# junhuihe2000/FLGP

Hardware: AMD Instinct MI355X
Metric: points/sec through k-NN->Laplacian->trunc-SVD->heat-cov, n=1e6 d=16 K=200 (higher is better)
Workload: dtype f64

## Files before the change

flgp_amd/csrc/sparse.hip:

```cpp
#include "common.h"

namespace flgp {

__global__ __launch_bounds__(256) void csc_hist_kernel(const int *__restrict__ ell_idx, long nnz, int s,
                                                       int chunk, int *__restrict__ hist) {
  extern __shared__ int lh[];
  for (int j = threadIdx.x; j < s; j += blockDim.x) lh[j] = 0;
  __syncthreads();
  const long e0 = (long)blockIdx.x * chunk;
  long e1 = e0 + chunk;
  if (e1 > nnz) e1 = nnz;
  for (long e = e0 + threadIdx.x; e < e1; e += blockDim.x) atomicAdd(&lh[ell_idx[e]], 1);
  __syncthreads();
  int *out = hist + (size_t)blockIdx.x * s;
  for (int j = threadIdx.x; j < s; j += blockDim.x) out[j] = lh[j];
}

__global__ void csc_colscan_kernel(int *__restrict__ hist, int nchunks, int s, int *__restrict__ tot) {
  const int j = blockIdx.x * blockDim.x + threadIdx.x;
  if (j >= s) return;
  int run = 0;
  constexpr int CB = 16;
  int c = 0;
  for (; c + CB <= nchunks; c += CB) {
    int h[CB];
#pragma unroll
    for (int u = 0; u < CB; ++u) h[u] = hist[(size_t)(c + u) * s + j];
#pragma unroll
    for (int u = 0; u < CB; ++u) { hist[(size_t)(c + u) * s + j] = run; run += h[u]; }
  }
  for (; c < nchunks; ++c) {
    const int h = hist[(size_t)c * s + j];
    hist[(size_t)c * s + j] = run;
    run += h;
  }
  tot[j] = run;
}

__global__ __launch_bounds__(1024) void csc_scan_kernel(const int *__restrict__ tot, int s, int *__restrict__ colptr) {
  __shared__ int part[1024];
  const int t = threadIdx.x;
  const int per = (s + 1023) / 1024;
  const int lo = t * per, hi = (lo + per < s) ? lo + per : s;
  int sum = 0;
  for (int j = lo; j < hi; ++j) sum += tot[j];
  part[t] = sum;
  __syncthreads();
  for (int off = 1; off < 1024; off <<= 1) {
    int v = (t >= off) ? part[t - off] : 0;
    __syncthreads();
    part[t] += v;
    __syncthreads();
  }
  int run = (t == 0) ? 0 : part[t - 1];
  for (int j = lo; j < hi; ++j) { colptr[j] = run; run += tot[j]; }
  if (t == 1023) colptr[s] = part[1023];
}

__global__ __launch_bounds__(64) void csc_scatter_kernel(const int *__restrict__ ell_idx, long nnz, int s,
                                                         int chunk, int nbits, const int *__restrict__ hist,
                                                         const int *__restrict__ colptr, int *__restrict__ pos) {
  extern __shared__ int cur[];
  const int lane = threadIdx.x;
  for (int j = lane; j < s; j += 64) cur[j] = 0;
  __syncthreads();
  const int *hoff = hist + (size_t)blockIdx.x * s;
  const long e0 = (long)blockIdx.x * chunk;
  long e1 = e0 + chunk;
  if (e1 > nnz) e1 = nnz;
  const unsigned long long lt = (lane == 0) ? 0ull : (~0ull >> (64 - lane));
  for (long eb = e0; eb < e1; eb += 64) {
    const long e = eb + lane;
    const bool act = e < e1;
    const int col = act ? ell_idx[e] : 0;
    unsigned long long m = __ballot(act);
    for (int b = 0; b < nbits; ++b) {
      const bool bit = (col >> b) & 1;
      const unsigned long long bal = __ballot(bit);
      m &= bit ? bal : ~bal;
    }
    if (act) {
      const int rank = __popcll(m & lt);
      const int base = cur[col];
      pos[(size_t)colptr[col] + hoff[col] + base + rank] = (int)e;
      if (rank == 0) cur[col] = base + __popcll(m);
    }
    __syncthreads();
  }
}

constexpr int COLSUM_CHUNK = 1024;

template <bool WIN>
__global__ __launch_bounds__(64) void colsum_chunk_kernel(const int *__restrict__ ell_idx, const double *__restrict__ val,
                                                          int n, int r, int s, int nbits, double *__restrict__ part, int wmax,
                                                          int direct) {
  extern __shared__ double bins[];
  const int lane = threadIdx.x;
  const int w0 = WIN ? (int)blockIdx.y * wmax : 0;
  const int wn = WIN ? ((s - w0 < wmax) ? s - w0 : wmax) : s;
  for (int j = lane; j < wn; j += 64) bins[j] = 0.0;
  __syncthreads();
  const long i0 = (long)blockIdx.x * COLSUM_CHUNK;
  const long i1 = (i0 + COLSUM_CHUNK < n) ? i0 + COLSUM_CHUNK : n;
  const long e0 = i0 * r, e1 = i1 * r;
  if (direct) {
    constexpr int CU = 8;
    for (long eb = e0; eb < e1; eb += 64 * CU) {
      int cq[CU];
      double vq[CU];
#pragma unroll
      for (int u = 0; u < CU; ++u) {
        const long e = eb + 64 * u + lane;
        const long ec = e < e1 ? e : e1 - 1;
        cq[u] = ell_idx[ec];
        vq[u] = val[ec];
      }
#pragma unroll
      for (int u = 0; u < CU; ++u) {
        const bool on = eb + 64 * u + lane < e1 && (!WIN || (unsigned)(cq[u] - w0) < (unsigned)wn);
        const int bin = on ? cq[u] - w0 : 0;
        if (on) __builtin_amdgcn_ds_atomic_fadd_f64((__attribute__((address_space(3))) double *)&bins[bin], vq[u]);
      }
    }
    __syncthreads();
    double *outd = part + (size_t)blockIdx.x * s + w0;
    for (int j = lane; j < wn; j += 64) outd[j] = bins[j];
    return;
  }
  const unsigned long long lt = (lane == 0) ? 0ull : (~0ull >> (64 - lane));
  long e = e0 + lane;
  int col = (e < e1) ? ell_idx[e] : 0;
  double v = (e < e1) ? val[e] : 0.0;
  for (long eb = e0; eb < e1; eb += 64) {
    const long en = eb + 64 + lane;
    const int coln = (en < e1) ? ell_idx[en] : 0;
    const double vn = (en < e1) ? val[en] : 0.0;
    const bool act = eb + lane < e1 && (!WIN || (unsigned)(col - w0) < (unsigned)wn);
    unsigned long long m = __ballot(act);
    for (int b = 0; b < nbits; ++b) {
      const bool bit = (col >> b) & 1;
      const unsigned long long bal = __ballot(bit);
      m &= bit ? bal : ~bal;
    }
    const int rank = act ? __popcll(m & lt) : -1;
    for (int k = 0; __ballot(rank == k) != 0ull; ++k)
      if (rank == k)
        __builtin_amdgcn_ds_atomic_fadd_f64((__attribute__((address_space(3))) double *)&bins[col - w0], v);
    col = coln; v = vn;
  }
  __syncthreads();
  double *out = part + (size_t)blockIdx.x * s + w0;
  for (int j = lane; j < wn; j += 64) out[j] = bins[j];
}

__global__ void colsum_reduce_kernel(const double *__restrict__ part, int nchunks, int s, double *__restrict__ colsum) {
  const int j = blockIdx.x * blockDim.x + threadIdx.x;
  if (j >= s) return;
  double acc = 0.0;
  int c = 0;
  for (; c + 32 <= nchunks; c += 32) {
    double p[32];
#pragma unroll
    for (int u = 0; u < 32; ++u) p[u] = part[(size_t)(c + u) * s + j];
#pragma unroll
    for (int u = 0; u < 32; ++u) acc += p[u];
  }
  for (; c + 8 <= nchunks; c += 8) {
    double p[8];
#pragma unroll
    for (int u = 0; u < 8; ++u) p[u] = part[(size_t)(c + u) * s + j];
#pragma unroll
    for (int u = 0; u < 8; ++u) acc += p[u];
  }
  for (; c < nchunks; ++c) acc += part[(size_t)c * s + j];
  colsum[j] = acc;
}

__global__ void col_scale_kernel(const int *__restrict__ ell_idx, double *__restrict__ val, long nnz,
                                 const double *__restrict__ colsum, const double *__restrict__ num_class,
                                 int mode) {
  const long e = (long)blockIdx.x * blockDim.x + threadIdx.x;
  if (e >= nnz) return;
  const int j = ell_idx[e];
  const double c = colsum[j];
  double v = val[e];
  if (mode == 0) {
    v = v * (1.0 / (c + 1e-9));
    if (num_class) v = v * num_class[j];
  } else {
    v = v * (1.0 / __builtin_sqrt(__builtin_fabs(c) + 1e-9));
  }
  val[e] = v;
}

__global__ __launch_bounds__(256) void row_normalize_kernel(double *__restrict__ val, int n, int r,
                                                            const int *__restrict__ idx = nullptr,
                                                            const double *__restrict__ colsum = nullptr,
                                                            const double *__restrict__ num_class = nullptr) {
  extern __shared__ double rn_rows[];
  const long i0 = (long)blockIdx.x * 256;
  const int rows = (n - i0 < 256) ? (int)(n - i0) : 256;
  double *g = val + (size_t)i0 * r;
  const int cnt = rows * r;
  if (idx) {
    const int *gi = idx + (size_t)i0 * r;
    for (int e = threadIdx.x; e < cnt; e += 256) {
      const int j = gi[e];
      double v = g[e];
      v = v * (1.0 / (colsum[j] + 1e-9));
      if (num_class) v = v * num_class[j];
      rn_rows[e] = v;
    }
  } else
  for (int e = threadIdx.x; e < cnt; e += 256) rn_rows[e] = g[e];
  __syncthreads();
  if ((int)threadIdx.x < rows) {
    double *row = rn_rows + (size_t)threadIdx.x * r;
    double rs = 0.0;
    for (int a = 0; a < r; ++a) rs += row[a];
    const double inv = 1.0 / (rs + 1e-9);
    for (int a = 0; a < r; ++a) row[a] = inv * row[a];
  }
  __syncthreads();
  for (int e = threadIdx.x; e < cnt; e += 256) g[e] = rn_rows[e];
}

__global__ __launch_bounds__(256) void extend_scale_kernel(const int *__restrict__ idx, double *__restrict__ val, int n, int r,
                                                           const double *__restrict__ c1, const double *__restrict__ num_class,
                                                           const double *__restrict__ c2) {
  extern __shared__ double es_rows[];
  const long i0 = (long)blockIdx.x * 256;
  const int rows = (n - i0 < 256) ? (int)(n - i0) : 256;
  double *g = val + (size_t)i0 * r;
  const int *gi = idx + (size_t)i0 * r;
  const int cnt = rows * r;
  if (c1) {
    for (int e = threadIdx.x; e < cnt; e += 256) {
      const int j = gi[e];
      double v = g[e];
      v = v * (1.0 / (c1[j] + 1e-9));
      if (num_class) v = v * num_class[j];
      es_rows[e] = v;
    }
  } else
  for (int e = threadIdx.x; e < cnt; e += 256) es_rows[e] = g[e];
  __syncthreads();
  if ((int)threadIdx.x < rows) {
    double *row = es_rows + (size_t)threadIdx.x * r;
    double rs = 0.0;
    for (int a = 0; a < r; ++a) rs += row[a];
    const double inv = 1.0 / (rs + 1e-9);
    for (int a = 0; a < r; ++a) row[a] = inv * row[a];
  }
  __syncthreads();
  for (int e = threadIdx.x; e < cnt; e += 256)
    g[e] = es_rows[e] * (1.0 / __builtin_sqrt(__builtin_fabs(c2[gi[e]]) + 1e-9));
}

constexpr int GRAM_PF = 4;

template <int LPR, bool WIN>
__global__ __launch_bounds__(64) void gram_kernel(const int *__restrict__ ell_idx, const double *__restrict__ val,
                                                  int s, int r, double inv_r, const int *__restrict__ colptr,
                                                  const int *__restrict__ pos, double *__restrict__ G, int ldg, int wmax) {
  extern __shared__ double acc[];
  constexpr int RPG = 64 / LPR;
  constexpr int NG = 64 / RPG;
  const int lane = threadIdx.x;
  const int j1 = blockIdx.x;
  const int w0 = WIN ? (int)blockIdx.y * wmax : 0;
  const int wn = WIN ? ((s - w0 < wmax) ? s - w0 : wmax) : s;
  for (int j = lane; j < wn; j += 64) acc[j] = 0.0;
  __syncthreads();
  const int sub = lane / LPR;
  const int a = lane % LPR;
  const bool slot_ok = a < r;
  const int ac = slot_ok ? a : 0;
  const int p0 = colptr[j1], p1 = colptr[j1 + 1];
  int epos = (p0 + lane < p1) ? pos[p0 + lane] : 0;
  for (int pc = p0; pc < p1; pc += 64) {
    const int pn = pc + 64 + lane;
    const int epos_next = (pn < p1) ? pos[pn] : 0;
    const int cnt = (p1 - pc < 64) ? p1 - pc : 64;
    struct Grp { int j2; double v, vj; bool act; };
    auto fetch = [&](int g) {
      Grp o;
      const int slot = g * RPG + sub;
      o.act = slot_ok && slot < cnt;
      const int e = __shfl(epos, slot & 63, 64);
      const int ee = o.act ? e : 0;
      const int row = (int)(((double)ee + 0.5) * inv_r);
      const size_t rowbase = (size_t)row * r;
      o.j2 = ell_idx[rowbase + ac];
      o.v = val[rowbase + ac];
      o.vj = val[ee];
      return o;
    };
    auto apply = [&](const Grp &o) {
      const double prod = o.vj * o.v;
      const bool on = o.act && (!WIN || (unsigned)(o.j2 - w0) < (unsigned)wn);
      const int bin = on ? o.j2 - w0 : 0;
      if (on) __builtin_amdgcn_ds_atomic_fadd_f64((__attribute__((address_space(3))) double *)&acc[bin], prod);
    };
    Grp cur[GRAM_PF], nxt[GRAM_PF];
#pragma unroll
    for (int u = 0; u < GRAM_PF; ++u) cur[u] = fetch(u);
    for (int g0 = 0; g0 < NG; g0 += GRAM_PF) {
      if (g0 * RPG >= cnt) break;
#pragma unroll
      for (int u = 0; u < GRAM_PF; ++u) nxt[u] = fetch(g0 + GRAM_PF + u);
#pragma unroll
      for (int u = 0; u < GRAM_PF; ++u) apply(cur[u]);
#pragma unroll
      for (int u = 0; u < GRAM_PF; ++u) cur[u] = nxt[u];
    }
    epos = epos_next;
  }
  __syncthreads();
  double *out = G + (size_t)j1 * ldg + w0;
  for (int j = lane; j < wn; j += 64) out[j] = acc[j];
}

__global__ __launch_bounds__(256) void u_recover_kernel(const int *__restrict__ ell_idx,
                                                        const double *__restrict__ val, int n, int r,
                                                        const double *__restrict__ V, int ldv,
                                                        const double *__restrict__ eig, int K, double scale,
                                                        double *__restrict__ out, int ldo) {
  const long i = (long)blockIdx.x * blockDim.x + threadIdx.x;
  if (i >= n) return;
  const int k0 = blockIdx.y * 8;
  double acc[8];
#pragma unroll
  for (int kk = 0; kk < 8; ++kk) acc[kk] = 0.0;
  for (int a = 0; a < r; ++a) {
    const int id = ell_idx[(size_t)i * r + a];
    const double va = val[(size_t)i * r + a];
#pragma unroll
    for (int kk = 0; kk < 8; ++kk)
      if (k0 + kk < K) acc[kk] += va * V[(size_t)(k0 + kk) * ldv + id];
  }
#pragma unroll
  for (int kk = 0; kk < 8; ++kk) {
    const int k = k0 + kk;
    if (k < K) {
      const double ev = eig[k];
      const double sigma = __builtin_sqrt(ev > 0.0 ? ev : 0.0);
      out[(size_t)k * ldo + i] = sigma > 0.0 ? (acc[kk] / sigma) * scale : 0.0;
    }
  }
}

__global__ void transpose_v_kernel(const double *__restrict__ V, int ldv, int s, int K, double *__restrict__ Vt) {
  __shared__ double t[32][33];
  const int j0 = blockIdx.x * 32, k0 = blockIdx.y * 32;
  const int tx = threadIdx.x & 31, ty = threadIdx.x >> 5;
  for (int kk = ty; kk < 32; kk += 8) {
    const int j = j0 + tx, k = k0 + kk;
    t[kk][tx] = (j < s && k < K) ? V[(size_t)k * ldv + j] : 0.0;
  }
  __syncthreads();
  for (int jj = ty; jj < 32; jj += 8) {
    const int j = j0 + jj, k = k0 + tx;
    if (j < s && k < K) Vt[(size_t)j * K + k] = t[tx][jj];
  }
}

#ifndef U_RECOVER_UNROLL
#define U_RECOVER_UNROLL 8
#endif
__global__ __launch_bounds__(256) void u_recover_tiled_kernel(const int *__restrict__ ell_idx,
                                                              const double *__restrict__ val, int n, int r,
                                                              const double *__restrict__ Vt,
                                                              const double *__restrict__ eig, int K, double scale,
                                                              double *__restrict__ out, int ldo) {
  __shared__ double tile[64][65];
  const int tid = threadIdx.x, lane = tid & 63, wave = tid >> 6;
  const long i0 = (long)blockIdx.x * 64;
  const int k0 = blockIdx.y * 64;
  const int k = k0 + lane;
  const bool kok = k < K;
  double sigma = 1.0;
  if (kok) { const double ev = eig[k]; sigma = __builtin_sqrt(ev > 0.0 ? ev : 0.0); }
  constexpr int UR = U_RECOVER_UNROLL;
  const double inv_guard = kok ? 1.0 : 0.0;
  const int kk = kok ? k : 0;
  for (int il = wave * 16; il < wave * 16 + 16; il += UR) {
    double acc[UR];
#pragma unroll
    for (int u = 0; u < UR; ++u) acc[u] = 0.0;
    for (int a = 0; a < r; ++a) {
      double v[UR], z[UR];
#pragma unroll
      for (int u = 0; u < UR; ++u) {
        const long i = (i0 + il + u < n) ? i0 + il + u : n - 1;
        z[u] = val[(size_t)i * r + a];
        v[u] = Vt[(size_t)ell_idx[(size_t)i * r + a] * K + kk];
      }
#pragma unroll
      for (int u = 0; u < UR; ++u) acc[u] += z[u] * v[u];
    }
#pragma unroll
    for (int u = 0; u < UR; ++u) tile[lane][il + u] = sigma > 0.0 ? ((acc[u] * inv_guard) / sigma) * scale : 0.0;
  }
  __syncthreads();
  const int i = tid & 63;
  if (i0 + i < n)
    for (int kq = tid >> 6; kq < 64; kq += 4)
      if (k0 + kq < K) out[(size_t)(k0 + kq) * ldo + i0 + i] = tile[kq][i];
}

template <int KPL, int ROWS>
__global__ __launch_bounds__(256) void u_recover_wide_kernel(const int *__restrict__ ell_idx,
                                                             const double *__restrict__ val, int n, int r,
                                                             const double *__restrict__ Vt,
                                                             const double *__restrict__ eig, int K, double scale,
                                                             double *__restrict__ out, int ldo) {
  typedef double vec_t __attribute__((ext_vector_type(KPL)));
  constexpr int KT = 64 * KPL, RPW = ROWS / 4;
  constexpr int UR = (RPW < U_RECOVER_UNROLL) ? RPW : U_RECOVER_UNROLL;
  __shared__ double tile[KT][ROWS + 1];
  const int tid = threadIdx.x, lane = tid & 63, wave = tid >> 6;
  const long i0 = (long)blockIdx.x * ROWS;
  const int k0 = blockIdx.y * KT;
  const int k = k0 + KPL * lane;
  const bool kok = k < K;
  double sg[KPL];
#pragma unroll
  for (int c = 0; c < KPL; ++c) { const double e = kok ? eig[k + c] : 1.0; sg[c] = __builtin_sqrt(e > 0.0 ? e : 0.0); }
  const double inv_guard = kok ? 1.0 : 0.0;
  const int kk = kok ? k : 0;
  for (int il = wave * RPW; il < wave * RPW + RPW; il += UR) {
    vec_t acc[UR];
#pragma unroll
    for (int u = 0; u < UR; ++u)
#pragma unroll
      for (int c = 0; c < KPL; ++c) acc[u][c] = 0.0;
    for (int a = 0; a < r; ++a) {
      vec_t v[UR];
      double z[UR];
#pragma unroll
      for (int u = 0; u < UR; ++u) {
        const long i = (i0 + il + u < n) ? i0 + il + u : n - 1;
        z[u] = val[(size_t)i * r + a];
        v[u] = *(const vec_t *)(Vt + (size_t)ell_idx[(size_t)i * r + a] * K + kk);
      }
#pragma unroll
      for (int u = 0; u < UR; ++u)
#pragma unroll
        for (int c = 0; c < KPL; ++c) acc[u][c] += z[u] * v[u][c];
    }
#pragma unroll
    for (int u = 0; u < UR; ++u)
#pragma unroll
      for (int c = 0; c < KPL; ++c)
        tile[KPL * lane + c][il + u] = sg[c] > 0.0 ? ((acc[u][c] * inv_guard) / sg[c]) * scale : 0.0;
  }
  __syncthreads();
  for (int e = tid; e < KT * ROWS; e += 256) {
    const int kq = e / ROWS, i = e % ROWS;
    if (k0 + kq < K && i0 + i < n) out[(size_t)(k0 + kq) * ldo + i0 + i] = tile[kq][i];
  }
}

#ifndef U_RECOVER_LDS_THREADS
#define U_RECOVER_LDS_THREADS 1024
#endif
#ifndef U_RECOVER_LDS_MIN_N
#define U_RECOVER_LDS_MIN_N 10000
#endif
constexpr int U_LDS_BYTES = 163840;

static int u_lds_width(int s) {
  const long w = s >= 1 ? (long)U_LDS_BYTES / (8L * s) : 0;
  return w > 4 ? 4 : (int)w;
}

template <int W>
__global__ __launch_bounds__(256) void transpose_v_slices_kernel(const double *__restrict__ V, int ldv, int s, int K,
                                                                 double *__restrict__ Vts) {
  const int j = blockIdx.x * 256 + threadIdx.x, sl = blockIdx.y;
  if (j >= s) return;
  double *o = Vts + ((size_t)sl * s + j) * W;
#pragma unroll
  for (int c = 0; c < W; ++c) {
    const int k = sl * W + c;
    o[c] = k < K ? V[(size_t)k * ldv + j] : 0.0;
  }
}

template <int W> __device__ __forceinline__ int u_lds_slot(int q) { return W == 4 ? q ^ (((q >> 5) & 1) << 1) : q; }

template <int W>
__global__ __launch_bounds__(U_RECOVER_LDS_THREADS) void u_recover_lds_kernel(const int *__restrict__ ell_idx,
                                                                              const double *__restrict__ val, int n, int r, int s,
                                                                              const double *__restrict__ Vts,
                                                                              const double *__restrict__ eig, int K, double scale,
                                                                              double *__restrict__ out, int ldo, int rows_per_range) {
  typedef double d2u __attribute__((ext_vector_type(2), aligned(8)));
  typedef int i2u __attribute__((ext_vector_type(2), aligned(4)));
  typedef double d2 __attribute__((ext_vector_type(2)));
  extern __shared__ __attribute__((aligned(16))) double u_slice[];
  const int tid = threadIdx.x, T = blockDim.x, sl = blockIdx.y;
  const double *src = Vts + (size_t)sl * s * W;
  for (int q = tid; q < s * W; q += T) u_slice[u_lds_slot<W>(q)] = src[q];
  double sg[W];
#pragma unroll
  for (int c = 0; c < W; ++c) {
    const int k = sl * W + c;
    const double e = k < K ? eig[k] : 0.0;
    sg[c] = __builtin_sqrt(e > 0.0 ? e : 0.0);
  }
  __syncthreads();
  const long i_lo = (long)blockIdx.x * rows_per_range;
  const long i_hi = (i_lo + rows_per_range < n) ? i_lo + rows_per_range : n;
  const long last_pair = (long)n * r - 2;
  struct Chunk { double z0[4], z1[4]; int j0[4], j1[4]; };
  auto fetch = [&](long i, int ch) {
    Chunk c;
#pragma unroll
    for (int u = 0; u < 4; ++u) {
      const int a = 8 * ch + 2 * u;
      long b = (i < i_hi && a < r) ? i * r + a : i_lo * r;
      b = b < last_pair ? b : last_pair;
      const d2u z = *(const d2u *)(val + b);
      const i2u j = *(const i2u *)(ell_idx + b);
      c.z0[u] = z[0]; c.z1[u] = z[1];
      c.j0[u] = j[0]; c.j1[u] = j[1];
    }
    return c;
  };
  auto gather = [&](const Chunk &cur, int u, int h, bool moved, double &z, double (&v)[W]) {
    const bool up = h || moved;
    const int id = up ? cur.j1[u] : cur.j0[u];
    z = up ? cur.z1[u] : cur.z0[u];
    if constexpr (W == 4) {
      const int x = ((id >> 3) & 1) << 1;
      const d2 lo = *(const d2 *)&u_slice[id * 4 + x], hi = *(const d2 *)&u_slice[id * 4 + (x ^ 2)];
      v[0] = lo[0]; v[1] = lo[1]; v[2] = hi[0]; v[3] = hi[1];
    } else if constexpr (W == 2) {
      const d2 lo = *(const d2 *)&u_slice[id * 2];
      v[0] = lo[0]; v[1] = lo[1];
    } else {
#pragma unroll
      for (int c = 0; c < W; ++c) v[c] = u_slice[id * W + c];
    }
  };
  double acc[W];
#pragma unroll
  for (int c = 0; c < W; ++c) acc[c] = 0.0;
  const int nch = (r + 7) >> 3;
  auto apply = [&](const Chunk &cur, long i, int ch) {
    const int left = r - ch * 8;
    if (left >= 8) {
      double z[8], v[8][W];
#pragma unroll
      for (int e = 0; e < 8; ++e) gather(cur, e >> 1, e & 1, false, z[e], v[e]);
#pragma unroll
      for (int e = 0; e < 8; ++e)
#pragma unroll
        for (int c = 0; c < W; ++c) acc[c] += z[e] * v[e][c];
    } else {
#pragma unroll
      for (int u = 0; u < 4; ++u) {
        const bool moved = i * r + ch * 8 + 2 * u > last_pair;
#pragma unroll
        for (int h = 0; h < 2; ++h)
          if (2 * u + h < left) {
            double z, v[W];
            gather(cur, u, h, moved, z, v);
#pragma unroll
            for (int c = 0; c < W; ++c) acc[c] += z * v[c];
          }
      }
    }
    if (ch == nch - 1) {
      if (i < i_hi) {
#pragma unroll
        for (int c = 0; c < W; ++c) {
          const int k = sl * W + c;
          if (k < K) out[(size_t)k * ldo + i] = sg[c] > 0.0 ? (acc[c] / sg[c]) * scale : 0.0;
        }
      }
#pragma unroll
      for (int c = 0; c < W; ++c) acc[c] = 0.0;
    }
  };
  const long nit = i_hi > i_lo ? (i_hi - i_lo + T - 1) / T : 0;
  const long steps = nit * nch;
  long ia = i_lo + tid; int cha = 0;
  auto next = [&](long &i, int &ch) { if (++ch == nch) { ch = 0; i += T; } };
  Chunk A = fetch(ia, cha), B;
  for (long t = 0; t < steps; t += 2) {
    long ib = ia; int chb = cha; next(ib, chb);
    B = fetch(ib, chb);
    apply(A, ia, cha);
    ia = ib; cha = chb; next(ia, cha);
    A = fetch(ia, cha);
    if (t + 1 < steps) apply(B, ib, chb);
  }
}

__global__ void values_out_kernel(const double *__restrict__ eig, int K, int root, double *__restrict__ values) {
  const int k = blockIdx.x * blockDim.x + threadIdx.x;
  if (k >= K) return;
  const double ev = eig[k] > 0.0 ? eig[k] : 0.0;
  values[k] = root ? __builtin_sqrt(ev) : ev;
}

struct CscPlan {
  int nchunks, chunk, nbits;
  size_t hist_bytes, tot_bytes;
};

static CscPlan csc_plan(long nnz, int s) {
  CscPlan p;
  long nc = (nnz + 2047) / 2048;
  if (nc > 2048) nc = 2048;
  if (nc < 1) nc = 1;
  long chunk = (nnz + nc - 1) / nc;
  chunk = (chunk + 63) / 64 * 64;
  if (chunk < 64) chunk = 64;
  p.chunk = (int)chunk;
  p.nchunks = (int)((nnz + chunk - 1) / chunk);
  if (p.nchunks < 1) p.nchunks = 1;
  p.nbits = 1;
  while ((1 << p.nbits) < s) ++p.nbits;
  p.hist_bytes = sizeof(int) * (size_t)p.nchunks * s;
  p.tot_bytes = sizeof(int) * (size_t)s;
  return p;
}

}

using namespace flgp;

extern "C" size_t flgp_dev_csc_workspace(int n, int s, int r) {
  const CscPlan p = csc_plan((long)n * r, s);
  return p.hist_bytes + p.tot_bytes + 256;
}

extern "C" int flgp_dev_csc_build(void *stream, const int *d_ell_idx, int n, int s, int r, int *d_colptr,
                                  int *d_pos, void *d_work, size_t work_bytes) {
  hipStream_t st = (hipStream_t)stream;
  const long nnz = (long)n * r;
  FLGP_REQUIRE(nnz < 2147483647L, "CSC: n*r = %ld does not fit int32 positions", nnz);
  FLGP_REQUIRE(s >= 1 && s <= FLGP_SMAX, "CSC: kernels are built for s <= %d (got %d)", FLGP_SMAX, s);
  FLGP_REQUIRE(work_bytes >= flgp_dev_csc_workspace(n, s, r), "CSC: workspace too small");
  const CscPlan p = csc_plan(nnz, s);
  int *hist = (int *)d_work;
  int *tot = (int *)((char *)d_work + p.hist_bytes);
  const size_t lds = sizeof(int) * (size_t)s;
  if (lds > 48 * 1024) {
    FLGP_HIP(hipFuncSetAttribute((const void *)csc_hist_kernel, hipFuncAttributeMaxDynamicSharedMemorySize, (int)lds));
    FLGP_HIP(hipFuncSetAttribute((const void *)csc_scatter_kernel, hipFuncAttributeMaxDynamicSharedMemorySize, (int)lds));
  }
  ProfScope ps("csc_build", st, 12.0 * (double)nnz);
  hipLaunchKernelGGL(csc_hist_kernel, dim3(p.nchunks), dim3(256), lds, st, d_ell_idx, nnz, s, p.chunk, hist);
  FLGP_TRY(check_launch("csc_hist_kernel"));
  hipLaunchKernelGGL(csc_colscan_kernel, dim3(ceil_div(s, 256)), dim3(256), 0, st, hist, p.nchunks, s, tot);
  FLGP_TRY(check_launch("csc_colscan_kernel"));
  hipLaunchKernelGGL(csc_scan_kernel, dim3(1), dim3(1024), 0, st, tot, s, d_colptr);
  FLGP_TRY(check_launch("csc_scan_kernel"));
  hipLaunchKernelGGL(csc_scatter_kernel, dim3(p.nchunks), dim3(64), lds, st, d_ell_idx, nnz, s, p.chunk, p.nbits,
                     hist, d_colptr, d_pos);
  return check_launch("csc_scatter_kernel");
}

static int lds_window(int s) {
  const int forced = tuning("sparse_window", 0);
  if (forced > 0 && forced < s) return forced;
  return s <= 20000 ? s : 16384;
}

extern "C" size_t flgp_dev_colsum_workspace(int n, int s) {
  return sizeof(double) * (size_t)ceil_div(n > 0 ? n : 1, COLSUM_CHUNK) * (size_t)s + 256;
}

extern "C" int flgp_dev_colsum(void *stream, const int *d_ell_idx, const double *d_ell_val, int n, int r, int s,
                               double *d_colsum, void *d_work, size_t work_bytes) {
  hipStream_t st = (hipStream_t)stream;
  FLGP_REQUIRE(n >= 0 && r >= 1 && s >= 1 && s <= FLGP_SMAX, "colsum: need 1 <= s <= %d (got %d)", FLGP_SMAX, s);
  FLGP_REQUIRE(work_bytes >= flgp_dev_colsum_workspace(n, s), "colsum: workspace too small");
  const int nchunks = ceil_div(n > 0 ? n : 1, COLSUM_CHUNK);
  int nbits = 1;
  while ((1 << nbits) < s) ++nbits;
  const int wmax = lds_window(s);
  const size_t lds = sizeof(double) * (size_t)wmax;
  const void *fn = wmax < s ? (const void *)colsum_chunk_kernel<true> : (const void *)colsum_chunk_kernel<false>;
  if (lds > 48 * 1024) FLGP_HIP(hipFuncSetAttribute(fn, hipFuncAttributeMaxDynamicSharedMemorySize, (int)lds));
  ProfScope ps("colsum_kernel", st, 12.0 * (double)n * r);
  if (wmax < s)
    hipLaunchKernelGGL(colsum_chunk_kernel<true>, dim3(nchunks, ceil_div(s, wmax)), dim3(64), lds, st, d_ell_idx, d_ell_val, n, r, s,
                       nbits, (double *)d_work, wmax, tuning("colsum_direct", 1));
  else
    hipLaunchKernelGGL(colsum_chunk_kernel<false>, dim3(nchunks), dim3(64), lds, st, d_ell_idx, d_ell_val, n, r, s, nbits,
                       (double *)d_work, wmax, tuning("colsum_direct", 1));
  FLGP_TRY(check_launch("colsum_chunk_kernel"));
  hipLaunchKernelGGL(colsum_reduce_kernel, dim3(ceil_div(s, 64)), dim3(64), 0, st, (const double *)d_work, nchunks, s, d_colsum);
  return check_launch("colsum_reduce_kernel");
}

extern "C" int flgp_dev_col_scale(void *stream, const int *d_ell_idx, double *d_ell_val, int n, int r,
                                  const double *d_colsum, const double *d_num_class, int mode) {
  FLGP_REQUIRE(mode == 0 || mode == 1, "col_scale: mode must be 0 or 1");
  const long nnz = (long)n * r;
  if (nnz == 0) return FLGP_OK;
  hipLaunchKernelGGL(col_scale_kernel, dim3(ceil_div(nnz, 256)), dim3(256), 0, (hipStream_t)stream, d_ell_idx,
                     d_ell_val, nnz, d_colsum, d_num_class, mode);
  return check_launch("col_scale_kernel");
}

extern "C" int flgp_dev_row_normalize(void *stream, double *d_ell_val, int n, int r) {
  if (n == 0) return FLGP_OK;
  FLGP_REQUIRE(r >= 1 && r <= FLGP_RMAX, "row_normalize: r = %d outside 1..%d", r, FLGP_RMAX);
  const size_t lds = sizeof(double) * 256 * (size_t)r;
  if (lds > 48 * 1024)
    FLGP_HIP(hipFuncSetAttribute((const void *)row_normalize_kernel, hipFuncAttributeMaxDynamicSharedMemorySize, (int)lds));
  hipLaunchKernelGGL(row_normalize_kernel, dim3(ceil_div(n, 256)), dim3(256), lds, (hipStream_t)stream, d_ell_val,
                     n, r);
  return check_launch("row_normalize_kernel");
}

extern "C" int flgp_dev_col_scale_row_normalize(void *stream, const int *d_ell_idx, double *d_ell_val, int n, int r,
                                                const double *d_colsum, const double *d_num_class) {
  FLGP_REQUIRE(r >= 1 && r <= FLGP_RMAX && d_ell_idx && d_ell_val && d_colsum, "col_scale_row_normalize: bad arguments");
  if (n == 0) return FLGP_OK;
  const size_t lds = sizeof(double) * 256 * (size_t)r;
  if (lds > 48 * 1024)
    FLGP_HIP(hipFuncSetAttribute((const void *)row_normalize_kernel, hipFuncAttributeMaxDynamicSharedMemorySize, (int)lds));
  hipLaunchKernelGGL(row_normalize_kernel, dim3(ceil_div(n, 256)), dim3(256), lds, (hipStream_t)stream, d_ell_val, n, r, d_ell_idx,
                     d_colsum, d_num_class);
  return check_launch("row_normalize_kernel");
}

extern "C" int flgp_dev_extend_scale(void *stream, const int *d_ell_idx, double *d_ell_val, int n, int r,
                                     const double *d_colsum_gl, const double *d_num_class, const double *d_colsum_spectrum) {
  FLGP_REQUIRE(r >= 1 && r <= FLGP_RMAX && n >= 0 && d_ell_idx && d_ell_val && d_colsum_spectrum, "extend_scale: bad arguments");
  if (n == 0) return FLGP_OK;
  const size_t lds = sizeof(double) * 256 * (size_t)r;
  if (lds > 48 * 1024)
    FLGP_HIP(hipFuncSetAttribute((const void *)extend_scale_kernel, hipFuncAttributeMaxDynamicSharedMemorySize, (int)lds));
  hipLaunchKernelGGL(extend_scale_kernel, dim3(ceil_div(n, 256)), dim3(256), lds, (hipStream_t)stream, d_ell_idx, d_ell_val, n, r,
                     d_colsum_gl, d_num_class, d_colsum_spectrum);
  return check_launch("extend_scale_kernel");
}

extern "C" int flgp_dev_gram(void *stream, const int *d_ell_idx, const double *d_ell_val, int n, int s, int r,
                             const int *d_colptr, const int *d_pos, double *dG, int ldg) {
  (void)n;
  FLGP_REQUIRE(s >= 1 && s <= FLGP_SMAX, "Gram: need 1 <= s <= %d (got %d)", FLGP_SMAX, s);
  FLGP_REQUIRE(r >= 1 && r <= FLGP_RMAX && ldg >= s, "Gram: bad r / ldg");
  const int wmax = lds_window(s);
  const size_t lds = sizeof(double) * (size_t)wmax;
  const bool win = wmax < s;
  const void *fn = r <= 16 ? (win ? (const void *)gram_kernel<16, true> : (const void *)gram_kernel<16, false>)
                           : (win ? (const void *)gram_kernel<32, true> : (const void *)gram_kernel<32, false>);
  if (lds > 48 * 1024) FLGP_HIP(hipFuncSetAttribute(fn, hipFuncAttributeMaxDynamicSharedMemorySize, (int)lds));
  ProfScope ps("gram_kernel", (hipStream_t)stream, 12.0 * (double)n * r + 8.0 * (double)s * s);
  const dim3 grid(s, win ? ceil_div(s, wmax) : 1);
#define GRAM_LAUNCH(LPRv, WINv)                                                                                                \
  hipLaunchKernelGGL((gram_kernel<LPRv, WINv>), grid, dim3(64), lds, (hipStream_t)stream, d_ell_idx, d_ell_val, s, r,         \
                     1.0 / (double)r, d_colptr, d_pos, dG, ldg, wmax)
  if (r <= 16) { if (win) GRAM_LAUNCH(16, true); else GRAM_LAUNCH(16, false); }
  else { if (win) GRAM_LAUNCH(32, true); else GRAM_LAUNCH(32, false); }
#undef GRAM_LAUNCH
  return check_launch("gram_kernel");
}

__global__ __launch_bounds__(256) void sym_pack_kernel(const double *__restrict__ G, int ldg, int s, double *__restrict__ packed) {
  const int j = blockIdx.y;
  const int i = blockIdx.x * 256 + threadIdx.x;
  if (i <= j) packed[(size_t)j * (j + 1) / 2 + i] = G[(size_t)j * ldg + i];
}
__global__ __launch_bounds__(256) void sym_unpack_kernel(const double *__restrict__ packed, int s, double *__restrict__ G, int ldg) {
  __shared__ double tile[32][33];
  const int ti = blockIdx.x, tj = blockIdx.y;
  if (ti > tj) return;
  const int tx = threadIdx.x & 31, ty = threadIdx.x >> 5;
  for (int c = ty; c < 32; c += 8) {
    const int i = ti * 32 + tx, j = tj * 32 + c;
    double v = 0.0;
    if (i < s && j < s) {
      v = (i <= j) ? packed[(size_t)j * (j + 1) / 2 + i] : packed[(size_t)i * (i + 1) / 2 + j];
      G[(size_t)j * ldg + i] = v;
    }
    tile[c][tx] = v;
  }
  __syncthreads();
  if (ti == tj) return;
  for (int c = ty; c < 32; c += 8) {
    const int i = tj * 32 + tx, j = ti * 32 + c;
    if (i < s && j < s) G[(size_t)j * ldg + i] = tile[tx][c];
  }
}

extern "C" int flgp_dev_sym_pack(void *stream, const double *dG, int ldg, int s, double *d_packed) {
  FLGP_REQUIRE(s >= 1 && ldg >= s, "sym_pack: bad shape");
  hipLaunchKernelGGL(sym_pack_kernel, dim3(ceil_div(s, 256), s), dim3(256), 0, (hipStream_t)stream, dG, ldg, s, d_packed);
  return check_launch("sym_pack_kernel");
}
extern "C" int flgp_dev_sym_unpack(void *stream, const double *d_packed, int s, double *dG, int ldg) {
  FLGP_REQUIRE(s >= 1 && ldg >= s, "sym_unpack: bad shape");
  const int nt = ceil_div(s, 32);
  hipLaunchKernelGGL(sym_unpack_kernel, dim3(nt, nt), dim3(256), 0, (hipStream_t)stream, d_packed, s, dG, ldg);
  return check_launch("sym_unpack_kernel");
}

extern "C" size_t flgp_dev_u_recover_workspace(int s, int K) {
  const int w = u_lds_width(s);
  const size_t cols = w >= 1 && K >= 1 ? (size_t)ceil_div(K, w) * w : (size_t)(K > 0 ? K : 0);
  return sizeof(double) * (size_t)(s > 0 ? s : 0) * cols + 256;
}

extern "C" int flgp_dev_u_recover_route(int n, int r, int s, int K, int has_work) {
  if (!has_work) return 0;
  if (u_lds_width(s) >= 1 && n >= U_RECOVER_LDS_MIN_N && (long)n * r >= 2) return 4;
  return K % 4 == 0 ? 3 : K % 2 == 0 ? 2 : 1;
}

static int num_cus() {
  static int cus[16] = {0};
  int dev = 0;
  if (hipGetDevice(&dev) != hipSuccess || dev < 0 || dev >= 16) return 256;
  if (!cus[dev]) {
    int c = 0;
    cus[dev] = (hipDeviceGetAttribute(&c, hipDeviceAttributeMultiprocessorCount, dev) == hipSuccess && c > 0) ? c : 256;
  }
  return cus[dev];
}

template <int W>
static int u_recover_lds_launch(hipStream_t st, const int *d_ell_idx, const double *d_ell_val, int n, int r, const double *dV,
                                int ldv, int s, const double *d_eig, int K, double scale, double *d_vectors, int ldo,
                                double *d_work) {
  const int slices = ceil_div(K, W);
  hipLaunchKernelGGL((transpose_v_slices_kernel<W>), dim3(ceil_div(s, 256), slices), dim3(256), 0, st, dV, ldv, s, K, d_work);
  FLGP_TRY(check_launch("transpose_v_slices_kernel"));
  int ranges = num_cus() / slices;
  if (ranges < 1) ranges = 1;
  int rows = ceil_div(ceil_div(n, ranges), 64) * 64;
  ranges = ceil_div(n, rows);
  const size_t lds = sizeof(double) * (size_t)s * W;
  if (lds > 48 * 1024)
    FLGP_HIP(hipFuncSetAttribute((const void *)u_recover_lds_kernel<W>, hipFuncAttributeMaxDynamicSharedMemorySize, (int)lds));
  hipLaunchKernelGGL((u_recover_lds_kernel<W>), dim3(ranges, slices), dim3(U_RECOVER_LDS_THREADS), lds, st, d_ell_idx, d_ell_val,
                     n, r, s, d_work, d_eig, K, scale, d_vectors, ldo, rows);
  return FLGP_OK;
}

extern "C" int flgp_dev_u_recover(void *stream, const int *d_ell_idx, const double *d_ell_val, int n, int r,
                                  const double *dV, int ldv, int s, const double *d_eig, int K, double scale,
                                  int root, double *d_vectors, int ldo, double *d_values_out, double *d_work) {
  hipStream_t st = (hipStream_t)stream;
  FLGP_REQUIRE(r >= 1 && r <= FLGP_RMAX && K >= 1 && ldo >= n, "u_recover: bad shape");
  if (n > 0) {
    ProfScope ps("u_recover_kernel", st, 12.0 * (double)n * r + 8.0 * (double)s * K + 8.0 * (double)n * K);
    const int route = flgp_dev_u_recover_route(n, r, s, K, d_work != nullptr);
    if (route == 4) {
      switch (u_lds_width(s)) {
#define U_LDS_CASE(Wv)                                                                                                         \
  case Wv: FLGP_TRY(u_recover_lds_launch<Wv>(st, d_ell_idx, d_ell_val, n, r, dV, ldv, s, d_eig, K, scale, d_vectors, ldo, d_work)); break
        U_LDS_CASE(1); U_LDS_CASE(2); U_LDS_CASE(3);
        default: U_LDS_CASE(4);
#undef U_LDS_CASE
      }
    } else if (d_work) {
      hipLaunchKernelGGL(transpose_v_kernel, dim3(ceil_div(s, 32), ceil_div(K, 32)), dim3(256), 0, st, dV, ldv, s, K,
                         d_work);
      if (K % 4 == 0) {
        hipLaunchKernelGGL((u_recover_wide_kernel<4, 32>), dim3(ceil_div(n, 32), ceil_div(K, 256)), dim3(256), 0, st, d_ell_idx,
                           d_ell_val, n, r, d_work, d_eig, K, scale, d_vectors, ldo);
      } else if (K % 2 == 0) {
        hipLaunchKernelGGL((u_recover_wide_kernel<2, 64>), dim3(ceil_div(n, 64), ceil_div(K, 128)), dim3(256), 0, st, d_ell_idx,
                           d_ell_val, n, r, d_work, d_eig, K, scale, d_vectors, ldo);
      } else {
        hipLaunchKernelGGL(u_recover_tiled_kernel, dim3(ceil_div(n, 64), ceil_div(K, 64)), dim3(256), 0, st, d_ell_idx,
                           d_ell_val, n, r, d_work, d_eig, K, scale, d_vectors, ldo);
      }
    } else {
      hipLaunchKernelGGL(u_recover_kernel, dim3(ceil_div(n, 256), ceil_div(K, 8)), dim3(256), 0, st, d_ell_idx,
                         d_ell_val, n, r, dV, ldv, d_eig, K, scale, d_vectors, ldo);
    }
    FLGP_TRY(check_launch("u_recover_kernel"));
  }
  if (d_values_out) {
    hipLaunchKernelGGL(values_out_kernel, dim3(ceil_div(K, 256)), dim3(256), 0, st, d_eig, K, root, d_values_out);
    FLGP_TRY(check_launch("values_out_kernel"));
  }
  return FLGP_OK;
}
```

Before: 39.38 million.

## Pipeline Gram kernel across chunks and pack rows densely for small r

Rewrites the Gram kernel inner loop as a continuous software pipeline. Each iteration applies the previous group's LDS atomics while issuing the next group's gathers, and position loads are prefetched two chunks ahead. It also adds an LPR=0 variant that packs 64/r rows per wavefront instead of padding each row to 16 or 32 lanes, chosen on the host when r is small, so fewer lanes sit idle. This costs more registers from the GF-deep queue, up to 16 groups, and adds a runtime-r index calculation.

```diff
diff --git a/flgp_amd/csrc/sparse.hip b/flgp_amd/csrc/sparse.hip
--- a/flgp_amd/csrc/sparse.hip
+++ b/flgp_amd/csrc/sparse.hip
@@ -258,38 +258,34 @@
     g[e] = es_rows[e] * (1.0 / __builtin_sqrt(__builtin_fabs(c2[gi[e]]) + 1e-9));
 }
 
-constexpr int GRAM_PF = 4;
-
 template <int LPR, bool WIN>
 __global__ __launch_bounds__(64) void gram_kernel(const int *__restrict__ ell_idx, const double *__restrict__ val,
                                                   int s, int r, double inv_r, const int *__restrict__ colptr,
                                                   const int *__restrict__ pos, double *__restrict__ G, int ldg, int wmax) {
   extern __shared__ double acc[];
-  constexpr int RPG = 64 / LPR;
-  constexpr int NG = 64 / RPG;
+  constexpr int GF = LPR ? 16 : 11;
   const int lane = threadIdx.x;
   const int j1 = blockIdx.x;
   const int w0 = WIN ? (int)blockIdx.y * wmax : 0;
   const int wn = WIN ? ((s - w0 < wmax) ? s - w0 : wmax) : s;
   for (int j = lane; j < wn; j += 64) acc[j] = 0.0;
   __syncthreads();
-  const int sub = lane / LPR;
-  const int a = lane % LPR;
-  const bool slot_ok = a < r;
-  const int ac = slot_ok ? a : 0;
+  const int lpr = LPR ? LPR : r;
+  const int rpg = 64 / lpr;
+  const int sub = lane / lpr;
+  const int a = lane - sub * lpr;
+  const bool slot_ok = a < r && sub < rpg;
+  const int ac = a < r ? a : 0;
   const int p0 = colptr[j1], p1 = colptr[j1 + 1];
-  int epos = (p0 + lane < p1) ? pos[p0 + lane] : 0;
-  for (int pc = p0; pc < p1; pc += 64) {
-    const int pn = pc + 64 + lane;
-    const int epos_next = (pn < p1) ? pos[pn] : 0;
-    const int cnt = (p1 - pc < 64) ? p1 - pc : 64;
+  if (p0 < p1) {
+    const int ng = (63 + rpg) / rpg;
+    const int step = (ng <= GF) ? 64 : GF * rpg;
+    auto positions = [&](int pb) { const int p = pb + lane; return pos[p < p1 ? p : p0]; };
     struct Grp { int j2; double v, vj; bool act; };
-    auto fetch = [&](int g) {
+    auto fetch = [&](int en, bool act) {
       Grp o;
-      const int slot = g * RPG + sub;
-      o.act = slot_ok && slot < cnt;
-      const int e = __shfl(epos, slot & 63, 64);
-      const int ee = o.act ? e : 0;
+      o.act = act;
+      const int ee = act ? en : 0;
       const int row = (int)(((double)ee + 0.5) * inv_r);
       const size_t rowbase = (size_t)row * r;
       o.j2 = ell_idx[rowbase + ac];
@@ -303,19 +299,25 @@
       const int bin = on ? o.j2 - w0 : 0;
       if (on) __builtin_amdgcn_ds_atomic_fadd_f64((__attribute__((address_space(3))) double *)&acc[bin], prod);
     };
-    Grp cur[GRAM_PF], nxt[GRAM_PF];
-#pragma unroll
-    for (int u = 0; u < GRAM_PF; ++u) cur[u] = fetch(u);
-    for (int g0 = 0; g0 < NG; g0 += GRAM_PF) {
-      if (g0 * RPG >= cnt) break;
-#pragma unroll
-      for (int u = 0; u < GRAM_PF; ++u) nxt[u] = fetch(g0 + GRAM_PF + u);
-#pragma unroll
-      for (int u = 0; u < GRAM_PF; ++u) apply(cur[u]);
-#pragma unroll
-      for (int u = 0; u < GRAM_PF; ++u) cur[u] = nxt[u];
-    }
-    epos = epos_next;
+    Grp q[GF];
+#pragma unroll
+    for (int u = 0; u < GF; ++u) q[u] = Grp{0, 0.0, 0.0, false};
+    int e1 = positions(p0);
+    asm volatile("" : "+v"(e1));
+    for (int pc = p0 - step; pc < p1; pc += step) {
+      const int e2 = positions(pc + 2 * step);
+      const int left = p1 - pc - step;
+      const int cnt = left < step ? left : step;
+      int en[GF];
+#pragma unroll
+      for (int u = 0; u < GF; ++u) en[u] = __shfl(e1, (u * rpg + sub) & 63, 64);
+#pragma unroll
+      for (int u = 0; u < GF; ++u) {
+        apply(q[u]);
+        q[u] = fetch(en[u], slot_ok && u * rpg + sub < cnt);
+      }
+      e1 = e2;
+    }
   }
   __syncthreads();
   double *out = G + (size_t)j1 * ldg + w0;
@@ -754,15 +756,18 @@
   const int wmax = lds_window(s);
   const size_t lds = sizeof(double) * (size_t)wmax;
   const bool win = wmax < s;
-  const void *fn = r <= 16 ? (win ? (const void *)gram_kernel<16, true> : (const void *)gram_kernel<16, false>)
-                           : (win ? (const void *)gram_kernel<32, true> : (const void *)gram_kernel<32, false>);
+  const int lpr = (64 / r > (r <= 16 ? 4 : 2)) ? 0 : (r <= 16 ? 16 : 32);
+  const void *fn = lpr == 0 ? (win ? (const void *)gram_kernel<0, true> : (const void *)gram_kernel<0, false>)
+                 : lpr == 16 ? (win ? (const void *)gram_kernel<16, true> : (const void *)gram_kernel<16, false>)
+                             : (win ? (const void *)gram_kernel<32, true> : (const void *)gram_kernel<32, false>);
   if (lds > 48 * 1024) FLGP_HIP(hipFuncSetAttribute(fn, hipFuncAttributeMaxDynamicSharedMemorySize, (int)lds));
   ProfScope ps("gram_kernel", (hipStream_t)stream, 12.0 * (double)n * r + 8.0 * (double)s * s);
   const dim3 grid(s, win ? ceil_div(s, wmax) : 1);
 #define GRAM_LAUNCH(LPRv, WINv)                                                                                                \
   hipLaunchKernelGGL((gram_kernel<LPRv, WINv>), grid, dim3(64), lds, (hipStream_t)stream, d_ell_idx, d_ell_val, s, r,         \
                      1.0 / (double)r, d_colptr, d_pos, dG, ldg, wmax)
-  if (r <= 16) { if (win) GRAM_LAUNCH(16, true); else GRAM_LAUNCH(16, false); }
+  if (lpr == 0) { if (win) GRAM_LAUNCH(0, true); else GRAM_LAUNCH(0, false); }
+  else if (lpr == 16) { if (win) GRAM_LAUNCH(16, true); else GRAM_LAUNCH(16, false); }
   else { if (win) GRAM_LAUNCH(32, true); else GRAM_LAUNCH(32, false); }
 #undef GRAM_LAUNCH
   return check_launch("gram_kernel");
```

Measured after the change: 39.98 million (median of 6 runs). +1.5%, better.
